# NTU-CompHydroMet-Lab/P2I-GAN-benchmark

Hardware: AMD Instinct MI355X
Metric: train frames/sec (128x128x16) (higher is better)
Workload: dtype f32

## Files before the change

### p2i-gan-benchmark_amd/csrc/glue.hip

```cpp
#include "common.h"

namespace p2i {

template <int T>
__global__ __launch_bounds__(256) void attn_fwd_kernel(const float* __restrict__ x, const float* __restrict__ w0,
                                                       const float* __restrict__ b0, const float* __restrict__ w1,
                                                       const float* __restrict__ b1, float* out, int B, int HW) {
  __shared__ float sw[2][T * T + T];
  for (int i = threadIdx.x; i < T * T; i += blockDim.x) { sw[0][i] = w0[i]; sw[1][i] = w1[i]; }
  for (int i = threadIdx.x; i < T; i += blockDim.x) { sw[0][T * T + i] = b0[i]; sw[1][T * T + i] = b1[i]; }
  __syncthreads();
  const int p = blockIdx.x * blockDim.x + threadIdx.x, b = blockIdx.y;
  if (p >= HW) return;
  float h[T];
#pragma unroll
  for (int t = 0; t < T; ++t) h[t] = x[((size_t)b * T + t) * HW + p];
#pragma unroll
  for (int l = 0; l < 2; ++l) {
    float n[T];
#pragma unroll
    for (int i = 0; i < T; ++i) {
      float g = sw[l][T * T + i];
#pragma unroll
      for (int j = 0; j < T; ++j) g += sw[l][i * T + j] * h[j];
      const float a = h[i] + h[i] * g;
      n[i] = a > 0.f ? a : 0.f;
    }
#pragma unroll
    for (int i = 0; i < T; ++i) h[i] = n[i];
  }
#pragma unroll
  for (int t = 0; t < T; ++t) out[((size_t)b * T + t) * HW + p] = h[t];
}

constexpr int ATTN_LIST = 32;

template <int T>
__global__ __launch_bounds__(256) void attn_bwd_kernel(const float* __restrict__ x, const float* __restrict__ w0,
                                                       const float* __restrict__ b0, const float* __restrict__ w1,
                                                       const float* __restrict__ b1, const float* __restrict__ dout,
                                                       float* dw0, float* db0, float* dw1, float* db1, int B, int HW, DetWs ws) {
  constexpr int NP = T * T + T;
  constexpr int NE = (2 * NP + 255) / 256;
  constexpr int PPT = (ATTN_LIST * T + 255) / 256;
  constexpr int H0 = 0, H1 = 1, DG2 = 2, DG1 = 3;
  __shared__ float sw[2][NP];
  __shared__ float swT[2][T * T];
  __shared__ float lst[ATTN_LIST][4][T];
  __shared__ int act[256];
  __shared__ int wave_cnt[4];
  for (int i = threadIdx.x; i < T * T; i += blockDim.x) {
    const float a = w0[i], c = w1[i];
    sw[0][i] = a; sw[1][i] = c;
// ... 363 lines not shown
}
__global__ void act_bwd_kernel(const float* __restrict__ dy, const float* __restrict__ y, int act, float* out, int64_t n4, int64_t n) {
  for (int64_t i = blockIdx.x * (int64_t)blockDim.x + threadIdx.x; i < n4; i += (int64_t)gridDim.x * blockDim.x) {
    const float4 g = reinterpret_cast<const float4*>(dy)[i], v = reinterpret_cast<const float4*>(y)[i];
    reinterpret_cast<float4*>(out)[i] = make_float4(act_grad(g.x, v.x, act), act_grad(g.y, v.y, act), act_grad(g.z, v.z, act), act_grad(g.w, v.w, act));
  }
  if (blockIdx.x == 0 && threadIdx.x < n - n4 * 4) {
    const int64_t i = n4 * 4 + threadIdx.x;
    out[i] = act_grad(dy[i], y[i], act);
  }
}
__global__ void add2_kernel(float* out, const float* __restrict__ a, const float* __restrict__ b, int64_t n4, int64_t n) {
  for (int64_t i = blockIdx.x * (int64_t)blockDim.x + threadIdx.x; i < n4; i += (int64_t)gridDim.x * blockDim.x) {
    const float4 x = reinterpret_cast<const float4*>(a)[i], y = reinterpret_cast<const float4*>(b)[i];
    reinterpret_cast<float4*>(out)[i] = make_float4(x.x + y.x, x.y + y.y, x.z + y.z, x.w + y.w);
  }
  if (blockIdx.x == 0) for (int64_t i = 4 * n4 + threadIdx.x; i < n; i += blockDim.x) out[i] = a[i] + b[i];
}
__global__ void axpy_kernel(float* y, const float* __restrict__ x, float a, int64_t n) {
  for (int64_t i = blockIdx.x * (int64_t)blockDim.x + threadIdx.x; i < n; i += (int64_t)gridDim.x * blockDim.x) y[i] += a * x[i];
}
__global__ void adam_kernel(float* p, const float* __restrict__ g, float* m, float* v, int64_t n, float step_size, float beta1,
                            float beta2, float eps, float bc2_sqrt) {
  for (int64_t i = blockIdx.x * (int64_t)blockDim.x + threadIdx.x; i < n; i += (int64_t)gridDim.x * blockDim.x) {
    const float gi = g[i];
    const float mi = m[i] + (gi - m[i]) * (1.f - beta1);
    const float vi = beta2 * v[i] + (1.f - beta2) * gi * gi;
    m[i] = mi; v[i] = vi;
    const float denom = sqrtf(vi) / bc2_sqrt + eps;
    p[i] = p[i] - step_size * (mi / denom);
  }
}

__global__ void adam_coef_kernel(int32_t* step_dev, float* coef, float lr, float beta1, float beta2) {
  const int step = step_dev[0] + 1;
  step_dev[0] = step;
  const double bc1 = 1.0 - pow((double)beta1, (double)step), bc2 = 1.0 - pow((double)beta2, (double)step);
  coef[0] = (float)((double)lr / bc1);
  coef[1] = (float)sqrt(bc2);
}
__global__ void adam_dev_kernel(float* p, const float* __restrict__ g, float* m, float* v, int64_t n, const float* __restrict__ coef,
                                float beta1, float beta2, float eps) {
  const float step_size = coef[0], bc2_sqrt = coef[1];
  for (int64_t i = blockIdx.x * (int64_t)blockDim.x + threadIdx.x; i < n; i += (int64_t)gridDim.x * blockDim.x) {
    const float gi = g[i];
    const float mi = m[i] + (gi - m[i]) * (1.f - beta1);
    const float vi = beta2 * v[i] + (1.f - beta2) * gi * gi;
    m[i] = mi; v[i] = vi;
    const float denom = sqrtf(vi) / bc2_sqrt + eps;
    p[i] = p[i] - step_size * (mi / denom);
  }
}

static inline int grid_for(int64_t n, int block = 256, int cap = 8192) {
  int64_t g = (n + block - 1) / block;
  return (int)(g < 1 ? 1 : (g > cap ? cap : g));
}

__global__ __launch_bounds__(256) void det_reduce_kernel(const float* __restrict__ part, int groups, int n, long long gs, long long ks, const DetSegs segs) {
  const int g = blockIdx.x * blockDim.x + threadIdx.x;
  if (g >= groups) return;
  const float* p = part + (long long)g * gs;
  float sacc = 0.f;
  int k = 0;
  for (; k + 8 <= n; k += 8) {
    float v[8];
#pragma unroll
    for (int u = 0; u < 8; ++u) v[u] = p[(long long)(k + u) * ks];
#pragma unroll
    for (int u = 0; u < 8; ++u) sacc += v[u];
  }
  for (; k < n; ++k) sacc += p[(long long)k * ks];
  int r = g;
#pragma unroll
  for (int i = 0; i < 4; ++i) {
    if (r < segs.len[i]) { segs.out[i][r] += sacc; return; }
    r -= segs.len[i];
  }
}
int det_reduce(const float* part, int groups, int n, long long gs, long long ks, const DetSegs& segs, hipStream_t s) {
  P2I_LAUNCH(det_reduce_kernel, dim3(ceil_div(groups, 256)), dim3(256), 0, s, part, groups, n, gs, ks, segs);
  return launch_status();
}
}
using namespace p2i;

extern "C" int p2i_attn_fwd(const float* x, const float* w0, const float* b0, const float* w1, const float* b1, float* out,
                            int B, int T, int HW, void* stream) {
  P2I_REQUIRE(x && w0 && b0 && w1 && b1 && out, "null pointer");
  P2I_REQUIRE(T == 8 || T == 16 || T == 32, "AttentionBlock kernels exist for T in {8, 16, 32}");
  const dim3 grid(ceil_div(HW, 256), B);
  hipStream_t s = (hipStream_t)stream;
  if (T == 16) P2I_LAUNCH(attn_fwd_kernel<16>, grid, dim3(256), 0, s, x, w0, b0, w1, b1, out, B, HW);
  else if (T == 32) P2I_LAUNCH(attn_fwd_kernel<32>, grid, dim3(256), 0, s, x, w0, b0, w1, b1, out, B, HW);
  else P2I_LAUNCH(attn_fwd_kernel<8>, grid, dim3(256), 0, s, x, w0, b0, w1, b1, out, B, HW);
  return launch_status();
}
extern "C" int p2i_attn_bwd(const float* x, const float* w0, const float* b0, const float* w1, const float* b1,
                            const float* dout, float* dw0, float* db0, float* dw1, float* db1, int B, int T, int HW, void* stream) {
  P2I_REQUIRE(x && w0 && b0 && w1 && b1 && dout && dw0 && db0 && dw1 && db1, "null pointer");
  P2I_REQUIRE(T == 8 || T == 16 || T == 32, "AttentionBlock kernels exist for T in {8, 16, 32}");
  int gx = ceil_div(HW, 256);
  const int want = 64 / (B < 64 ? B : 64) > 0 ? 64 / (B < 64 ? B : 64) : 1;
  if (gx > want) gx = want;
  const dim3 grid(gx, B);
  hipStream_t s = (hipStream_t)stream;
  const size_t nblk = (size_t)grid.x * grid.y;
  const DetWs ws = det_take(nblk * 2 * (size_t)(T * T + T), 1);
  if (T == 16) P2I_LAUNCH(attn_bwd_kernel<16>, grid, dim3(256), 0, s, x, w0, b0, w1, b1, dout, dw0, db0, dw1, db1, B, HW, ws);
// ... 83 lines not shown
  P2I_LAUNCH(bias_grad_kernel, dim3(C, chunks), dim3(256), 0, (hipStream_t)stream, dy, y_act, act, db, B, C, inner, ws);
  if (ws.part) return det_reduce(ws.part, C, chunks, chunks, 1, DetSegs{{db, nullptr, nullptr, nullptr}, {C, 0, 0, 0}}, (hipStream_t)stream);
  return launch_status();
}
extern "C" int p2i_act_bwd(const float* dy, const float* y, int act, float* out, int64_t n, void* stream) {
  P2I_REQUIRE(dy && y && out && n > 0, "null pointer");
  P2I_LAUNCH(act_bwd_kernel, dim3(grid_for(n / 4 + 1)), dim3(256), 0, (hipStream_t)stream, dy, y, act, out, n / 4, n);
  return launch_status();
}
extern "C" int p2i_act_bwd_bias(const float* dy, const float* y, int act, float* out, float* db, int B, int C, int64_t inner, void* stream) {
  P2I_REQUIRE(dy && y && out && db && B > 0 && C > 0 && inner > 0, "null pointer");
  P2I_REQUIRE((inner & 3) == 0 && (((uintptr_t)dy | (uintptr_t)y | (uintptr_t)out) & 15) == 0, "inner % 4 and 16-byte alignment");
  int chunks = (int)((inner / 4 + 2047) / 2048);
  if (chunks > 16) chunks = 16;
  const DetWs ws = det_take((size_t)C * B * chunks, 0);
  P2I_LAUNCH(act_bwd_bias_kernel, dim3(C, B, chunks), dim3(256), 0, (hipStream_t)stream, dy, y, act, out, db, C, inner / 4, ws);
  if (ws.part) return det_reduce(ws.part, C, B * chunks, B * chunks, 1, DetSegs{{db, nullptr, nullptr, nullptr}, {C, 0, 0, 0}}, (hipStream_t)stream);
  return launch_status();
}
extern "C" int p2i_axpy(float* y, const float* x, float a, int64_t n, void* stream) {
  P2I_REQUIRE(y && x, "null pointer");
  P2I_LAUNCH(axpy_kernel, dim3(grid_for(n)), dim3(256), 0, (hipStream_t)stream, y, x, a, n);
  return launch_status();
}
extern "C" int p2i_add2(float* out, const float* a, const float* b, int64_t n, void* stream) {
  P2I_REQUIRE(out && a && b && n >= 0, "null pointer");
  const bool al = (((uintptr_t)out | (uintptr_t)a | (uintptr_t)b) & 15) == 0;
  const int64_t n4 = al ? n / 4 : 0;
  P2I_LAUNCH(add2_kernel, dim3(grid_for(n4 + 1)), dim3(256), 0, (hipStream_t)stream, out, a, b, n4, n);
  return launch_status();
}
extern "C" int p2i_zero(float* p, int64_t n, void* stream) {
  P2I_REQUIRE(p && n >= 0, "null pointer");
  if (n > 0 && p2i::memset_async(p, 0, sizeof(float) * (size_t)n, (hipStream_t)stream) != hipSuccess) { set_error("memset failed"); return P2I_EINVAL; }
  return P2I_OK;
}
extern "C" int p2i_adam(float* p, const float* g, float* m, float* v, int64_t n, float lr, float beta1, float beta2, float eps,
                        int step, void* stream) {
  P2I_REQUIRE(p && g && m && v && step >= 1, "bad adam arguments");
  const double bc1 = 1.0 - pow((double)beta1, step), bc2 = 1.0 - pow((double)beta2, step);
  P2I_LAUNCH(adam_kernel, dim3(grid_for(n)), dim3(256), 0, (hipStream_t)stream, p, g, m, v, n, (float)(lr / bc1), beta1,
                     beta2, eps, (float)sqrt(bc2));
  return launch_status();
}

extern "C" int p2i_adam_dev(float* p, const float* g, float* m, float* v, int64_t n, float lr, float beta1, float beta2, float eps,
                            int32_t* step_dev, float* coef2, void* stream) {
  P2I_REQUIRE(p && g && m && v && step_dev && coef2, "bad adam arguments");
  P2I_LAUNCH(adam_coef_kernel, dim3(1), dim3(1), 0, (hipStream_t)stream, step_dev, coef2, lr, beta1, beta2);
  P2I_LAUNCH(adam_dev_kernel, dim3(grid_for(n)), dim3(256), 0, (hipStream_t)stream, p, g, m, v, n, coef2, beta1, beta2, eps);
  return launch_status();
}


namespace p2i {
__global__ __launch_bounds__(256) void assemble_batch_kernel(const uint8_t* __restrict__ fr, const uint8_t* __restrict__ mk,
                                                             float* __restrict__ frames, float* __restrict__ masked,
                                                             float* __restrict__ masks, long long n, long long mask_period) {
  const long long stride = (long long)gridDim.x * 256 * 4;
  for (long long i0 = ((long long)blockIdx.x * 256 + threadIdx.x) * 4; i0 < n; i0 += stride) {
#pragma unroll
    for (int q = 0; q < 4; ++q) {
      const long long i = i0 + q;
      if (i < n) {
        const float v = __fdiv_rn((float)fr[i], 255.0f);
        const float m = mk[i % mask_period] ? 1.0f : 0.0f;
        frames[i] = v;
        masks[i] = m;
        masked[i] = v * m;
      }
    }
  }
}
}

__global__ __launch_bounds__(256) void window_gather_kernel(const float* __restrict__ a, const float* __restrict__ b, float* __restrict__ wa,
                                                           float* __restrict__ wb, int L, int64_t HW4, int w0, int nw, int win, int step) {
  const int64_t per = (int64_t)win * HW4;
  for (int64_t i = blockIdx.x * 256ll + threadIdx.x; i < (int64_t)nw * per; i += (int64_t)gridDim.x * 256) {
    const int w = (int)(i / per);
    const int64_t r = i - (int64_t)w * per;
    const int k = (int)(r / HW4);
    const int64_t p = r - (int64_t)k * HW4;
    const int l = min((w0 + w) * step + k, L - 1);
    reinterpret_cast<float4*>(wa)[i] = reinterpret_cast<const float4*>(a)[(int64_t)l * HW4 + p];
    if (b) reinterpret_cast<float4*>(wb)[i] = reinterpret_cast<const float4*>(b)[(int64_t)l * HW4 + p];
  }
}
__global__ __launch_bounds__(256) void window_mean_kernel(const float* __restrict__ pw, float* __restrict__ out, int L, int64_t HW4, int nwin, int win,
                                                         int step, float scale) {
  for (int64_t i = blockIdx.x * 256ll + threadIdx.x; i < (int64_t)L * HW4; i += (int64_t)gridDim.x * 256) {
    const int l = (int)(i / HW4);
    const int64_t p = i - (int64_t)l * HW4;
    const int wlo = l - win + 1 > 0 ? (l - win + 1 + step - 1) / step : 0, whi = min(l / step, nwin - 1);
    float4 acc = make_float4(0.f, 0.f, 0.f, 0.f);
    for (int w = wlo; w <= whi; ++w) {
      const float4 v = reinterpret_cast<const float4*>(pw)[((int64_t)w * win + (l - w * step)) * HW4 + p];
      acc.x += v.x; acc.y += v.y; acc.z += v.z; acc.w += v.w;
    }
    const float c = fmaxf((float)(whi - wlo + 1), 1e-5f);
    acc.x = fmaxf(acc.x / c * scale, 0.f); acc.y = fmaxf(acc.y / c * scale, 0.f);
    acc.z = fmaxf(acc.z / c * scale, 0.f); acc.w = fmaxf(acc.w / c * scale, 0.f);
    reinterpret_cast<float4*>(out)[i] = acc;
  }
}
extern "C" int p2i_window_gather(const float* a, const float* b, float* wa, float* wb, int L, int64_t HW, int w0, int nw, int win, int step,
// ... 28 lines not shown
```

### p2i-gan-benchmark_amd/csrc/weights.hip

```cpp
#include <stdarg.h>
#include "common.h"

namespace p2i {

static thread_local char g_err[512] = "";
void set_error(const char* fmt, ...) {
  va_list ap;
  va_start(ap, fmt);
  vsnprintf(g_err, sizeof(g_err), fmt, ap);
  va_end(ap);
}

__device__ __forceinline__ int pad32(int v) { return (v + 31) & ~31; }

constexpr int FOLD_MAX_LAYERS = 16;
struct FoldBatch {
  const float* W[FOLD_MAX_LAYERS];
  const float* D[FOLD_MAX_LAYERS];
  const float* Dd[FOLD_MAX_LAYERS];
  float* a[FOLD_MAX_LAYERS];
  float* b[FOLD_MAX_LAYERS];
  const float* g[FOLD_MAX_LAYERS];
};

// ... 241 lines not shown
    if (b.div[L]) v = v / *b.div[L];
    if (b.f[L]) b.f[L][((size_t)tap * I + i) * pad32(O) + o] = v;
    if (b.d[L]) b.d[L][((size_t)tap * O + o) * pad32(I) + i] = v;
  }
}
__global__ void unpack_dot_batched_kernel(const PackBatch b, DetWs ws) {
  __shared__ float red[16];
  const int L = blockIdx.z, O = b.O[L], I = b.I[L], NT = b.NT[L];
  if (!b.div[L]) return;
  float acc = 0.f;
  const int n = O * I * NT;
  for (int idx = blockIdx.x * blockDim.x + threadIdx.x; idx < n; idx += gridDim.x * blockDim.x) {
    const int tap = idx % NT, i = (idx / NT) % I, o = idx / (NT * I);
    acc += b.g[L][((size_t)tap * I + i) * pad32(O) + o] * b.w[L][idx];
  }
  acc = block_sum(acc, red);
  if (ws.part) {
    if (threadIdx.x == 0) ws.part[(size_t)L * gridDim.x + blockIdx.x] = acc;
    return;
  }
  if (threadIdx.x == 0 && acc != 0.f) atomicAdd(b.dot[L], acc);
}
__global__ void unpack_batched_kernel(const PackBatch b) {
  const int L = blockIdx.z, O = b.O[L], I = b.I[L], NT = b.NT[L];
  for (int idx = blockIdx.x * blockDim.x + threadIdx.x; idx < O * I * NT; idx += gridDim.x * blockDim.x) {
    const int tap = idx % NT, i = (idx / NT) % I, o = idx / (NT * I);
    float g = b.g[L][((size_t)tap * I + i) * pad32(O) + o];
    if (b.div[L]) {
      const float sg = *b.div[L];
      g = g / sg - (*b.dot[L] / (sg * sg)) * b.u[L][o] * b.v[L][i * NT + tap];
    }
    if (b.accumulate) b.f[L][idx] += g; else b.f[L][idx] = g;
  }
}

constexpr int SN_MAX_LAYERS = 16;
struct SnBatch {
  const float* w[SN_MAX_LAYERS];
  float* u[SN_MAX_LAYERS];
  float* v[SN_MAX_LAYERS];
  float* sigma[SN_MAX_LAYERS];
  float* scratch[SN_MAX_LAYERS];
  float* usnap[SN_MAX_LAYERS];
  float* vsnap[SN_MAX_LAYERS];
  int O[SN_MAX_LAYERS], K[SN_MAX_LAYERS];
  int n;
};
__global__ __launch_bounds__(256) void sn_wtu_batched_kernel(const SnBatch b) {
  __shared__ float part[4][64];
  const int L = blockIdx.z, O = b.O[L], K = b.K[L];
  if ((int)blockIdx.x * 64 >= K) return;
  const float* w = b.w[L];
  const float* u = b.u[L];
  const int col = threadIdx.x & 63, rg = threadIdx.x >> 6, k = blockIdx.x * 64 + col;
  float acc = 0.f;
  if (k < K)
    for (int o = rg; o < O; o += 4) acc += w[(size_t)o * K + k] * u[o];
  part[rg][col] = acc;
  __syncthreads();
  if (rg == 0 && k < K) b.scratch[L][k] = part[0][col] + part[1][col] + part[2][col] + part[3][col];
}
__global__ void sn_wv_batched_kernel(const SnBatch b) {
  const int L = blockIdx.z, O = b.O[L], K = b.K[L];
  const int o = blockIdx.x * (blockDim.x >> 6) + (threadIdx.x >> 6), lane = threadIdx.x & 63;
  if (o >= O) return;
  const float* w = b.w[L];
  const float* v = b.v[L];
  float acc = 0.f;
  for (int k = lane; k < K; k += 64) acc += w[(size_t)o * K + k] * v[k];
  acc = wave_sum(acc);
  if (lane == 0) b.scratch[L][K + o] = acc;
}
__global__ void sn_finish_batched_kernel(const SnBatch b, int phase) {
  __shared__ float red[16];
  const int L = blockIdx.z, O = b.O[L], K = b.K[L];
  const float* in = phase == 0 ? b.scratch[L] : b.scratch[L] + K;
  const int n = phase == 0 ? K : O;
  if (phase == 2) {
    float acc = 0.f;
    for (int i = threadIdx.x; i < n; i += blockDim.x) acc += b.u[L][i] * in[i];
    acc = block_sum(acc, red);
    if (threadIdx.x == 0) *b.sigma[L] = acc;
    return;
  }
  float* out = phase == 0 ? b.v[L] : b.u[L];
  float* snap = phase == 0 ? b.vsnap[L] : b.usnap[L];
  float acc = 0.f;
  for (int i = threadIdx.x; i < n; i += blockDim.x) acc += in[i] * in[i];
  const float nrm = fmaxf(sqrtf(block_sum(acc, red)), 1e-12f);
  float dot = 0.f;
  for (int i = threadIdx.x; i < n; i += blockDim.x) {
    const float o = in[i] / nrm;
    out[i] = o;
    if (snap) snap[i] = o;
    dot += o * in[i];
  }
  if (phase == 1) {
    dot = block_sum(dot, red);
    if (threadIdx.x == 0) *b.sigma[L] = dot;
  }
}

static int fold_fwd_launch(const FoldBatch& fb, int n, int O, int I, hipStream_t s) {
  P2I_LAUNCH(fold_fwd_tile_batched_kernel, dim3(I / 32, O / 32, n), dim3(256), 0, s, fb, O, I);
  return launch_status();
}
static int fold_bwd_launch(const FoldBatch& fb, int n, int O, int I, hipStream_t s) {
  P2I_LAUNCH(fold_bwd_w_tile_batched_kernel, dim3(I / 32, O / 32, n), dim3(256), 0, s, fb, O, I);
  P2I_LAUNCH(fold_bwd_d_batched_kernel, dim3(I / 32, 1, n), dim3(256), 0, s, fb, O, I);
  return launch_status();
}
static int pack_launch(const PackBatch& b, int n, int maxn, hipStream_t s) {
  const int blocks = ceil_div(maxn, 256);
  P2I_LAUNCH(pack_batched_kernel, dim3(blocks > 512 ? 512 : blocks, 1, n), dim3(256), 0, s, b);
  return launch_status();
}
static int unpack_launch(const PackBatch& b, int n, int maxn, float* dots, hipStream_t s) {
  bool any_sigma = false;
  for (int i = 0; i < n; ++i) any_sigma = any_sigma || b.div[i] != nullptr;
  const int blocks = ceil_div(maxn, 256);
  if (any_sigma) {
    (void)p2i::memset_async(dots, 0, sizeof(float) * n, s);
// ... 174 lines not shown
```

### p2i-gan-benchmark_amd/p2igan_bench/_hip.py

```python
from __future__ import annotations

import ctypes as C
import os

_LIB_PATH = os.path.join(os.path.dirname(os.path.abspath(__file__)), "_lib", "libp2i_hip.so")
_lib = None

ACT_NONE, ACT_RELU, ACT_LEAKY, ACT_TANH = 0, 1, 2, 3


class ConvDesc(C.Structure):
    _fields_ = [(n, C.c_int) for n in
                ("B", "Cin", "Cout", "Ti", "Hi", "Wi", "To", "Ho", "Wo", "kt", "kh", "kw",
                 "st", "sh", "sw", "pt", "ph", "pw")]


class ConvSplit(C.Structure):
    _fields_ = [("w_split", C.c_void_p), ("w_scratch", C.c_void_p), ("src_planes", C.c_void_p), ("w_split_taps", C.c_int)]


class EvalInput(C.Structure):
    _fields_ = [("data", C.c_void_p)] + [(n, C.c_int) for n in ("dtype", "h", "w", "top", "left")]


# ... 107 lines not shown
    "p2i_krig_bins": [_P, _P, _P, _I, _I, _I, _I, _F64, _P, _P],
    "p2i_krig_fit": [_P, _I, _I, _I, _F64, _I, _P, _P, _P, _P, _P],
    "p2i_krig_factor": [_K, _P, _P],
    "p2i_krig_solve": [_K, _P, _P, _P, _P, _P],
    "p2i_krig_predict": [_K, _P, _P, _I, _I, _P, _P],
    "p2i_idw_all": [_P, _P, _P, _I, _I, _I, _I, _F, _P, _P],
    "p2i_krig_invert": [_P, _I, _I, _P, _P],
    "p2i_krig_variance": [_K, _P, _P, _I, _I, _P, _P],
    "p2i_krig_loo": [_K, _P, _P, _P, _P, _P, _P, _P],
    "p2i_krig_cs_spectrum": [_P, _P, _I, _I, _I, _I, _P, _P, _P, _P, _P],
    "p2i_krig_cs_noise": [C.c_uint64, _L, _I, _I, _I, _I, _P, _P],
    "p2i_krig_cs_fields": [_P, _P, _P, _P, C.c_uint64, _I, _I, _I, _I, _I, _I, _I, _I, _P, _P, _P],
    "p2i_krig_cs_weights": [_K, _P, _P, _P, _I, _I, _I, _P, _P, _P],
    "p2i_krig_cs_predict": [_K, _P, _P, _I, _I, _I, _P, _P],
    "p2i_stkrig_gather": [_P, _P, _P, _I, _I, _I, _I, _P, _P, _P, _P, _P],
    "p2i_stkrig_bins": [_P, _P, _P, _P, _I, _I, _I, _I, _I, _I, _F64, _P, _P],
    "p2i_stkrig_fit": [_P, _I, _I, _I, _I, _F64, _I, _P, _P, _P, _P, _P],
    "p2i_stkrig_factor": [_K, _P, _P, _P, _P],
    "p2i_stkrig_predict": [_P, _P, _P, _P, _P, _P, _P, _I, _I, _I, _I, _I, _I, _P, _P],
    "p2i_stkrig_gather_sites": [_P, _P, _P, _I, _I, _I, _I, _P, _P, _P, _P, _P, _P, _P, _P, _P, _P],
    "p2i_stkrig_site_gram": [_P, _I, _I, _P, _P],
    "p2i_stkrig_loso": [_K, _P, _P, _P, _P, _P, _P, _I, _I, _P, _P, _P],
    "p2i_lagkrig_velocity": [_P, _P, _P, _I, _I, _I, _I, _I, _I, _F64, _F64, _P, _P],
    "p2i_lagkrig_pick": [_P, _I, _I, _I, _F64, _P, _P, _P, _P, _P, _P, _P],
    "p2i_lkrig_predict": [_P, _P, _P, _P, _P, _I, _I, _I, _I, _I, _I, _I, _I, _P, _P, _P, _P, _P, _P, _P],
    "p2i_lkrig_loso": [_P, _P, _P, _P, _P, _I, _I, _I, _I, _I, _I, _P, _P, _P, _P, _P, _P],
    "p2i_idw_loo": [_P, _P, _P, _I, _I, _F, _P, _P],
    "p2i_loo_scores": [_P, _P, _P, _P, _I, _I, _P, _P, _P],
    "p2i_scale_fss": [_E, _E, _I, _I, _P, C.POINTER(C.c_double), _I, C.POINTER(C.c_int), _I, _I, _P, _P, _P],
    "p2i_scale_fss_merge": [_P, _L, _I, _P, _P],
    "p2i_scale_dft_rows": [_E, _I, _I, _I, _P, _I, _P, _P, _P, _P],
    "p2i_scale_dft_cols": [_P, _I, _I, _P, _P, _P],
    "p2i_scale_rings": [_P, _I, _I, _P, _P, _P, _P, _I, _P, _P],
    "p2i_scale_spectrum_merge": [_P, _P, _L, _I, _P, _P],
    "p2i_prob_record": [_I, _I, _I, _I, _I, C.POINTER(C.c_int), C.POINTER(C.c_int)],
    "p2i_prob_accumulate": [_E, _E, _F64, _E, _L, _I, _I, _P, _P, C.POINTER(C.c_double), C.POINTER(C.c_double), _I,
                            C.POINTER(C.c_double), _I, C.POINTER(C.c_double), _I, _I, _I, _I, _I, _P, _L, _P],
    "p2i_prob_merge": [_P, _L, _I, _I, _P, _P],
    "p2i_objects_quantize": [_E, _I, _I, _I, _P, C.POINTER(C.c_double), _I, _F64, _F64, _I, _P, _P, _P, _P],
    "p2i_objects_label": [_P, _I, _I, _I, _I, _I, _P, _P],
    "p2i_objects_count": [_P, _I, _P, _I, _I, _I, _P, _P, _P],
    "p2i_objects_scan": [_P, _L, _P, _P],
    "p2i_objects_fill": [_P, _I, _P, _I, _I, _I, _P, _L, _P, _P],
}

ENS_SIGNATURES = {
    "p2i_ens_abi_version": [],
    "p2i_ens_record": [_I, _I, _I, C.POINTER(C.c_int), C.POINTER(C.c_int)],
    "p2i_ens_points": [_E, _I, _L, _E, _L, _I, _I, _I, _P, C.POINTER(C.c_double), _I, C.POINTER(C.c_double), _I, _P, _L, _P],
    "p2i_ens_energy": [_E, _I, _L, _E, _L, _I, _I, _P, _P, _P],
    "p2i_ens_variogram": [_E, _I, _L, _E, _L, _I, _I, _P, C.POINTER(C.c_int), _I, _P, _P],
}


def lib_path() -> str:
    return _LIB_PATH


def load():
    global _lib
    if _lib is not None:
        return _lib
    if not os.path.exists(_LIB_PATH):
        raise RuntimeError(
            f"libp2i_hip.so not found at {_LIB_PATH}: build it with `python -c 'import __graft_entry__ as g; g.build()'` "
            "or `make -C p2i-gan-benchmark_amd/csrc`.  There is no CPU fallback for the product path.")
    lib = C.CDLL(os.environ.get("P2I_HIP_LIB") or _LIB_PATH)
    for table in (SIGNATURES, ENS_SIGNATURES):
        for name, args in table.items():
            fn = getattr(lib, name)
            fn.argtypes = args
            fn.restype = C.c_int
    lib.p2i_abi_version.restype = C.c_int
    lib.p2i_last_error.restype = C.c_char_p
    _lib = lib
    return lib


def check(rc: int, what: str):
    if rc != 0:
        msg = load().p2i_last_error().decode(errors="replace")
        raise RuntimeError(f"{what} failed (rc={rc}): {msg}")
```

### p2i-gan-benchmark_amd/p2igan_bench/engine.py

```python
from __future__ import annotations

from typing import Dict, List, Optional

import torch
import torch.distributed as dist
import torch.nn as nn

from . import ops
from .models import p2igan as net_fns
from .modules.losses import ReconstructionLoss, discriminator_loss, generator_adv_loss
from .parallel import BucketedAllReduce, FlatParams, allreduce_mean_, broadcast_module_state


class FusedAdam:

    def __init__(self, fp: FlatParams, lr: float, betas=(0.0, 0.99), eps: float = 1e-8):
        self.fp, self.lr, self.betas, self.eps = fp, lr, betas, eps
        self.m = torch.zeros_like(fp.flat)
        self.v = torch.zeros_like(fp.flat)
        self.step_count = 0
        self.step_dev = self.coef = None

    def use_device_step(self):
        self.step_dev = torch.tensor([self.step_count], device=self.fp.flat.device, dtype=torch.int32)
# ... 2 lines not shown
    def step(self):
        self.step_count += 1
        if self.step_dev is not None:
            ops.adam_step_dev(self.fp.flat, self.fp.grad, self.m, self.v, self.lr, self.betas[0], self.betas[1], self.eps,
                              self.step_dev, self.coef)
        else:
            ops.adam_step(self.fp.flat, self.fp.grad, self.m, self.v, self.lr, self.betas[0], self.betas[1], self.eps, self.step_count)
        inval = getattr(self.fp.module, "invalidate_weight_cache", None)
        if inval is not None:
            inval()

    def state_dict(self):
        return {"step": self.step_count, "exp_avg": self.m, "exp_avg_sq": self.v, "lr": self.lr, "betas": self.betas, "eps": self.eps}

    def load_state_dict(self, sd):
        self.step_count = int(sd["step"])
        self.m.copy_(sd["exp_avg"])
        self.v.copy_(sd["exp_avg_sq"])
        if self.step_dev is not None:
            self.step_dev.fill_(self.step_count)


def _allreduce_mean(buf: torch.Tensor, world: int):
    allreduce_mean_(buf, world, (lambda t, a: ops.axpy_(t, t, a - 1.0)) if buf.is_cuda else None)


class TrainEngine:
    def __init__(self, generator: nn.Module, discriminator: Optional[nn.Module], cfg: Dict, distributed: bool = False):
        self.G, self.D = generator, discriminator
        loss_cfg, opt_cfg = cfg["loss"], cfg["train"]["optimizer"]
        self.use_gan = bool(loss_cfg.get("use_gan", 0)) and discriminator is not None
        self.gan_type = loss_cfg.get("gan_loss", "hinge")
        self.real_label = loss_cfg.get("target_real_label", 1.0)
        self.fake_label = loss_cfg.get("target_fake_label", 0.0)
        self.adv_weight = loss_cfg.get("adversarial_weight", 0.01)
        self.rec_loss = ReconstructionLoss(k1_alpha=loss_cfg.get("k1_weight", 0.0))
        betas = (opt_cfg.get("beta1", 0.0), opt_cfg.get("beta2", 0.99))
        self.gp = FlatParams(self.G)
        self.opt_g = FusedAdam(self.gp, opt_cfg["lr"], betas)
        import os
        self.direct = os.environ.get("P2I_ENGINE_AUTOGRAD", "0") != "1" and isinstance(self.G, net_fns.P2IGenerator) and (
            discriminator is None or isinstance(discriminator, net_fns.P2IDiscriminator))
        self.dp = self.opt_d = None
        if self.use_gan:
            self.dp = FlatParams(self.D)
            self.opt_d = FusedAdam(self.dp, opt_cfg["lr"], betas)
        self.distributed = distributed and dist.is_initialized() and dist.get_world_size() > 1
        self.world = dist.get_world_size() if self.distributed else 1
        if self.distributed:
            self.broadcast_state()
        self.dp_overlap = os.environ.get("P2I_DP_OVERLAP", "1") != "0"
        self._level_ranges = None
        self.prep_overlap = os.environ.get("P2I_PREP_OVERLAP", "1") != "0"

    def broadcast_state(self):
        broadcast_module_state(self.G, self.gp)
        if self.D is not None:
            broadcast_module_state(self.D, self.dp)

    def level_range(self, lvl: int):
        if self._level_ranges is None:
            base, rngs = self.gp.grad.data_ptr(), []
            for blk in self.G.Decoder:
                ps = [p for p in blk.parameters() if p.requires_grad]
                lo = min((p.grad.data_ptr() - base) // 4 for p in ps)
                hi = max((p.grad.data_ptr() - base) // 4 + p.numel() for p in ps)
                if hi - lo != sum(p.numel() for p in ps):
                    raise RuntimeError("Decoder level is not one contiguous slice of the flat gradient buffer")
                rngs.append((int(lo), int(hi)))
            self._level_ranges = rngs
        return self._level_ranges[lvl]

    def capture(self, frames, masked, masks, warmup: int = 3, mode: str = "graph"):
        if self.distributed:
            raise RuntimeError("graph capture is for the single-GPU step")
        if not self.direct:
            raise RuntimeError("graph / tape capture replays the direct P2I-GAN step only; this engine runs the autograd step "
                               f"({type(self.G).__name__}), which stays eager")
        if mode not in ("graph", "tape"):
            raise ValueError(mode)
        for o in (self.opt_g, self.opt_d):
            if o is not None:
                o.use_device_step()
        self._static_in = [torch.empty_like(t) for t in (frames, masked, masks)]
        for dst, src in zip(self._static_in, (frames, masked, masks)):
            dst.copy_(src)
        side = torch.cuda.Stream()
        side.wait_stream(torch.cuda.current_stream())
        with torch.cuda.stream(side):
            for _ in range(warmup):
                self._step_impl(*self._static_in)
        torch.cuda.current_stream().wait_stream(side)
        self._graph = torch.cuda.CUDAGraph()
        self._tape = None
        import ctypes
        lib = ops._hip.load()
        with torch.cuda.graph(self._graph):
            if mode == "tape":
                ops._hip.check(lib.p2i_tape_begin(torch.cuda.current_stream().cuda_stream), "p2i_tape_begin")
            try:
                self._static_out = self._step_impl(*self._static_in)
            finally:
                if mode == "tape":
                    handle = ctypes.c_void_p()
                    ops._hip.check(lib.p2i_tape_end(ctypes.byref(handle)), "p2i_tape_end")
                    self._tape = handle
# ... 21 lines not shown

    def train_step(self, frames, masked, masks) -> Dict[str, torch.Tensor]:
        if getattr(self, "_graph", None) is not None:
            if tuple(frames.shape) == tuple(self._static_in[0].shape):
                for dst, src in zip(self._static_in, (frames, masked, masks)):
                    if dst.data_ptr() != src.data_ptr():
                        dst.copy_(src)
                if getattr(self, "_tape", None) is not None:
                    ops._hip.check(ops._hip.load().p2i_tape_replay(self._tape, torch.cuda.current_stream().cuda_stream), "p2i_tape_replay")
                else:
                    self._graph.replay()
                for o in (self.opt_g, self.opt_d):
                    if o is not None:
                        o.step_count += 1
                self.G.invalidate_weight_cache() if hasattr(self.G, "invalidate_weight_cache") else None
                return self._static_out
            return self._step_impl(frames, masked, masks)
        if self._auto_graph_wanted(frames):
            shp = tuple(frames.shape)
            self._same_shape_steps = getattr(self, "_same_shape_steps", 0) + 1 if getattr(self, "_last_shape", None) == shp else 0
            self._last_shape = shp
            if self._same_shape_steps >= self.AUTO_GRAPH_AFTER:
                import os
                self.capture(frames, masked, masks, warmup=0, mode="tape" if os.environ.get("P2I_AUTO_TAPE", "0") == "1" else "graph")
                return self.train_step(frames, masked, masks)
        return self._step_impl(frames, masked, masks)

    def _mark(self):
        if self.phase_marks is not None:
            e = torch.cuda.Event(enable_timing=True)
            e.record()
            self.phase_marks.append(e)

    phase_marks = None
    exchange_marks = None

    def _exchange(self, kind, fn):
        if self.exchange_marks is None or not self.gp.grad.is_cuda:
            return fn()
        e0, e1 = torch.cuda.Event(enable_timing=True), torch.cuda.Event(enable_timing=True)
        e0.record()
        out = fn()
        e1.record()
        self.exchange_marks.append((kind, e0, e1))
        return out

    def _step_direct(self, frames, masked, masks) -> Dict[str, torch.Tensor]:
        G, D = self.G, self.D
        self._mark()
        if not G.training:
            G.train()
        with torch.no_grad():
            side = net_fns._side_of(G, frames.device) if (self.prep_overlap and frames.is_cuda) else None
            real_box = [None]
            step_start = ops.mark_stream() if side is not None else None

            def enqueue_side_work():
                b_, t_, c_, h_, w_ = masked.shape
                gprep = side.run(lambda: net_fns.generator_prepare(G, b_, h_, w_), after=step_start)
                ready = side.mark()
                if self.use_gan:
                    if not D.training:
                        D.train()
                    dprep_f = side.run(lambda: net_fns.discriminator_prepare(D, tuple(masked.shape), frames.device, False, True, pool=True), after=step_start)
                    dprep_r = side.run(lambda: net_fns.discriminator_prepare(D, tuple(frames.shape), frames.device, False, True, pool=True), after=step_start)

                    def real_pass():
                        lr2, cr2 = net_fns.discriminator_forward(D, frames, need_x=False, need_p=True, pool=True, prep=dprep_r)
                        _, dlr2, _ = ops.gan_loss_d(lr2, lr2, self.gan_type, self.real_label, self.fake_label)
                        self.dp.zero_grad()
                        net_fns.discriminator_backward(D, cr2, dlr2, need_x=False, inplace=True, accumulate=False)
                        return lr2, None

                    real_box[0] = (dprep_f, side.run(real_pass, frames, after=step_start))
                return gprep, ready

            preds, S = net_fns.generator_forward(G, masked, masks, need_grad=True, after_head=enqueue_side_work if side is not None else None)
            dprep_f, real_out = real_box[0] if real_box[0] is not None else (None, None)
            if side is not None and self.use_gan:
                out3, dpred = side.run(lambda: ops.recloss(preds.contiguous(), frames.contiguous().float(), self.rec_loss.k1_alpha), preds, frames)
            else:
                out3, dpred = ops.recloss(preds.contiguous(), frames.contiguous().float(), self.rec_loss.k1_alpha)
            out = {"rec": out3[2], "pool": out3[0], "reg": out3[1]}
            self._mark()
            dgen = dpred
            loss_g = out3[2:3]
            if self.use_gan:
                if not D.training:
                    D.train()
                lf, cf = net_fns.discriminator_forward(D, preds, need_x=False, need_p=True, pool=True, prep=dprep_f)
            if side is not None:
                side.join()
            if self.use_gan:
                if real_out is not None and real_out[1] is None:
                    lr_ = real_out[0]
                    loss_d, _, dlf = ops.gan_loss_d(lr_, lf, self.gan_type, self.real_label, self.fake_label)
                    net_fns.discriminator_backward(D, cf, dlf, need_x=False, inplace=True, accumulate=True)
                    del cf
                else:
                    lr_, cr = real_out if real_out is not None else net_fns.discriminator_forward(D, frames, need_x=False, need_p=True, pool=True)
                    loss_d, dlr, dlf = ops.gan_loss_d(lr_, lf, self.gan_type, self.real_label, self.fake_label)
                    self.dp.zero_grad()
                    net_fns.discriminator_backward(D, cf, dlf, need_x=False, inplace=True, accumulate=False)
                    net_fns.discriminator_backward(D, cr, dlr, need_x=False, inplace=True, accumulate=True)
                    del cf, cr
                if self.distributed:
                    self._exchange("d", lambda: _allreduce_mean(self.dp.grad, self.world))
                self.opt_d.step()
                self._mark()
                lg, cg = net_fns.discriminator_forward(D, preds, need_x=True, need_p=False, pool=True)
                adv, dlg = ops.gan_loss_g(lg, self.adv_weight, self.gan_type, self.real_label)
                dgen, _, _, _ = net_fns.discriminator_backward(D, cg, dlg, need_x=True, needs=[False] * (2 * sum(map(len, D.layers())) + 1), dx_add=dpred)
                del cg
                loss_g = ops.add2(out3[2:3], adv)
                out.update(loss_d=loss_d.reshape(()), adv=adv.reshape(()), logits_real=lr_, logits_fake=lf)
            self.gp.zero_grad()
            if self.distributed and self.dp_overlap:
                bk = BucketedAllReduce(self.gp.grad, self.world, (lambda t, a: ops.axpy_(t, t, a - 1.0)) if self.gp.grad.is_cuda else None)
                net_fns.generator_backward(G, S, dgen, inplace=True, on_level_done=lambda lvl: bk.launch(*self.level_range(lvl)))
                del S
                self._exchange("g", bk.finish)
            else:
                net_fns.generator_backward(G, S, dgen, inplace=True)
                del S
                if self.distributed:
                    self._exchange("g", lambda: _allreduce_mean(self.gp.grad, self.world))
            self.opt_g.step()
            out.update(loss_g=loss_g.reshape(()), preds=preds)
            self._mark()
        return out

    def _step_impl(self, frames, masked, masks) -> Dict[str, torch.Tensor]:
        if self.direct:
            with ops.step_stream():
                return self._step_direct(frames, masked, masks)
        self._mark()
        self.G.train()
        preds = self.G(masked, masks)
        loss_g, parts = self.rec_loss(preds, frames, masks)
        out = {"rec": loss_g.detach(), "pool": parts["pool"].tensor(), "reg": parts["reg"].tensor()}
        self._mark()
        if self.use_gan:
            self.D.train()
            for p in self.dp.params:
                p.requires_grad_(True)
# ... 43 lines not shown
```

### p2i-gan-benchmark_amd/p2igan_bench/ops.py

```python
from __future__ import annotations

import ctypes as C
import math
from dataclasses import dataclass
from typing import Optional, Tuple

import torch

from . import _hip
from ._hip import ACT_LEAKY, ACT_NONE, ACT_RELU, ACT_TANH, ConvDesc


def _ptr(t: Optional[torch.Tensor]):
    return None if t is None else t.data_ptr()


_CUR_STREAM = None


def _stream():
    return _CUR_STREAM if _CUR_STREAM is not None else torch.cuda.current_stream().cuda_stream


class step_stream:
# ... 1087 lines not shown

def shock_map_bwd(x, dout, beta, eps):
    _chk_f32(x, dout)
    _same(x, dout, "shock_map_bwd")
    B, T, H, W, _, _ = _shock_dims(x, 1, 0, "shock_map")
    dx = torch.empty_like(x)
    scratch = torch.empty(3 * x.numel(), device=x.device, dtype=torch.float32)
    _hip.check(_hip.load().p2i_shock_map_bwd(_ptr(x), _ptr(dout), _ptr(dx), _ptr(scratch), B * T, H, W, float(beta), float(eps),
                                             _stream()), "p2i_shock_map_bwd")
    return dx


def shock_loss_fwd(pred, true, beta, pool, border, eps):
    _chk_f32(pred, true)
    _same(pred, true, "shock_loss_fwd")
    B, T, H, W, Hp, Wp = _shock_dims(pred, pool, border, "shock_map_loss")
    out = torch.empty((B, T, Hp - 2 * border, Wp - 2 * border), device=pred.device, dtype=torch.float32)
    _hip.check(_hip.load().p2i_shock_loss_fwd(_ptr(pred), _ptr(true), _ptr(out), B * T, H, W, int(pool), int(border), float(beta),
                                              float(eps), _stream()), "p2i_shock_loss_fwd")
    return out


def shock_loss_bwd(pred, true, dout, beta, pool, border, eps):
    _chk_f32(pred, true, dout)
    B, T, H, W, Hp, Wp = _shock_dims(pred, pool, border, "shock_map_loss")
    if tuple(dout.shape) != (B, T, Hp - 2 * border, Wp - 2 * border):
        raise RuntimeError(f"shock_loss_bwd: gradient {tuple(dout.shape)} does not match the loss tensor")
    dpred = torch.empty_like(pred)
    scratch = torch.empty(3 * B * T * Hp * Wp, device=pred.device, dtype=torch.float32)
    _hip.check(_hip.load().p2i_shock_loss_bwd(_ptr(pred), _ptr(true), _ptr(dout), _ptr(dpred), _ptr(scratch), B * T, H, W, int(pool),
                                              int(border), float(beta), float(eps), _stream()), "p2i_shock_loss_bwd")
    return dpred


def adam_step(p, g, m, v, lr, beta1, beta2, eps, step):
    lib = _hip.load()
    n = p.numel()
    if not (g.numel() == n and m.numel() == n and v.numel() == n):
        raise RuntimeError("adam_step: buffer size mismatch")
    _chk(p, g, m, v)
    _hip.check(lib.p2i_adam(_ptr(p), _ptr(g), _ptr(m), _ptr(v), n, lr, beta1, beta2, eps, step, _stream()), "p2i_adam")


def adam_step_dev(p, g, m, v, lr, beta1, beta2, eps, step_dev, coef):
    lib = _hip.load()
    n = p.numel()
    if not (g.numel() == n and m.numel() == n and v.numel() == n) or step_dev.dtype != torch.int32 or coef.numel() < 2:
        raise RuntimeError("adam_step_dev: bad buffers")
    _chk(p, g, m, v, step_dev, coef)
    _hip.check(lib.p2i_adam_dev(_ptr(p), _ptr(g), _ptr(m), _ptr(v), n, lr, beta1, beta2, eps, _ptr(step_dev), _ptr(coef), _stream()),
               "p2i_adam_dev")


def axpy_(y, x, a=1.0):
    lib = _hip.load()
    if y.numel() != x.numel():
        raise RuntimeError("axpy_: size mismatch")
    _chk(y, x)
    _hip.check(lib.p2i_axpy(_ptr(y), _ptr(x), float(a), y.numel(), _stream()), "p2i_axpy")
    return y


def zero_(t):
    lib = _hip.load()
    _chk(t)
    _hip.check(lib.p2i_zero(_ptr(t), t.numel(), _stream()), "p2i_zero")
    return t


def add2(a, b):
    lib = _hip.load()
    if a.shape != b.shape:
        raise RuntimeError("add2: shape mismatch")
    out = torch.empty_like(a)
    _chk(a, b)
    _hip.check(lib.p2i_add2(_ptr(out), _ptr(a), _ptr(b), a.numel(), _stream()), "p2i_add2")
    return out


def act_bwd(dy, y, act):
    lib = _hip.load()
    if dy.shape != y.shape:
        raise RuntimeError("act_bwd: shape mismatch")
    out = torch.empty_like(dy)
    _chk(dy, y)
    _hip.check(lib.p2i_act_bwd(_ptr(dy), _ptr(y), act, _ptr(out), dy.numel(), _stream()), "p2i_act_bwd")
    return out


def act_bwd_bias(dy, y, act, db_out=None):
    lib = _hip.load()
    det_ready(dy.device)
    B, Cc = dy.shape[0], dy.shape[1]
    inner = dy[0, 0].numel()
    if inner % 4:
        dz = act_bwd(dy, y, act)
        return dz, bias_grad(dz, out=db_out)
    out = torch.empty_like(dy)
    db = db_out if db_out is not None else zero_(torch.empty(Cc, device=dy.device, dtype=torch.float32))
    _chk(dy, y, db)
    _hip.check(lib.p2i_act_bwd_bias(_ptr(dy), _ptr(y), act, _ptr(out), _ptr(db), B, Cc, inner, _stream()), "p2i_act_bwd_bias")
    return out, db


def bias_grad(dy, y_act=None, act=ACT_NONE, out=None):
    lib = _hip.load()
# ... 1085 lines not shown
```

Measured before the change: 11460.

## Add vectorized ranged Adam, unroll spectral-norm matvecs, split discriminator side stream

Adds float4-vectorized ranged Adam entry points (host and device-step variants) with alignment-aware head/tail handling, though nothing in the shown code calls them yet. Rewrites the spectral-norm W^T u and W v kernels with deep unrolled load batches and fma to raise memory-level parallelism. The engine gets a separate side stream for discriminator prep, the real pass and the reconstruction loss, plus an event so the fake-branch forward waits only on its own prep. This aims for more overlap with generator work, at the cost of more streams and sync points.

```diff
diff --git a/include/p2i_opt.h b/include/p2i_opt.h
--- /dev/null
+++ b/include/p2i_opt.h
@@ -0,0 +1,18 @@
+#ifndef P2I_OPT_H
+#define P2I_OPT_H
+#include "p2i_hip.h"
+
+#ifdef __cplusplus
+extern "C" {
+#endif
+
+int p2i_opt_abi_version(void);
+int p2i_adam_range(float* p, const float* g, float* m, float* v, int64_t offset, int64_t n, float lr, float beta1, float beta2,
+                   float eps, int step, void* stream);
+int p2i_adam_range_dev(float* p, const float* g, float* m, float* v, int64_t offset, int64_t n, float lr, float beta1, float beta2,
+                       float eps, int32_t* step_dev, float* coef2, int advance, void* stream);
+
+#ifdef __cplusplus
+}
+#endif
+#endif
diff --git a/p2i-gan-benchmark_amd/csrc/glue.hip b/p2i-gan-benchmark_amd/csrc/glue.hip
--- a/p2i-gan-benchmark_amd/csrc/glue.hip
+++ b/p2i-gan-benchmark_amd/csrc/glue.hip
@@ -1,4 +1,5 @@
 #include "common.h"
+#include "p2i_opt.h"
 
 namespace p2i {
 
@@ -468,9 +469,54 @@
   }
 }
 
+__device__ __forceinline__ void adam_one(float& p, float gi, float& m, float& v, float step_size, float beta1, float beta2,
+                                         float eps, float bc2_sqrt) {
+#pragma clang fp contract(off)
+  const float mi = m + (gi - m) * (1.f - beta1);
+  const float vi = beta2 * v + (1.f - beta2) * gi * gi;
+  m = mi; v = vi;
+  const float denom = sqrtf(vi) / bc2_sqrt + eps;
+  p = fmaf(-step_size, mi / denom, p);
+}
+__global__ void adam_range_kernel(float* p, const float* __restrict__ g, float* m, float* v, int64_t n, int head, int64_t n4,
+                                  const float* __restrict__ coef, float step_size, float beta1, float beta2, float eps,
+                                  float bc2_sqrt) {
+  if (coef) { step_size = coef[0]; bc2_sqrt = coef[1]; }
+  float4* p4 = reinterpret_cast<float4*>(p + head);
+  const float4* g4 = reinterpret_cast<const float4*>(g + head);
+  float4* m4 = reinterpret_cast<float4*>(m + head);
+  float4* v4 = reinterpret_cast<float4*>(v + head);
+  for (int64_t i = blockIdx.x * (int64_t)blockDim.x + threadIdx.x; i < n4; i += (int64_t)gridDim.x * blockDim.x) {
+    float4 pi = p4[i], mi = m4[i], vi = v4[i];
+    const float4 gi = g4[i];
+    adam_one(pi.x, gi.x, mi.x, vi.x, step_size, beta1, beta2, eps, bc2_sqrt);
+    adam_one(pi.y, gi.y, mi.y, vi.y, step_size, beta1, beta2, eps, bc2_sqrt);
+    adam_one(pi.z, gi.z, mi.z, vi.z, step_size, beta1, beta2, eps, bc2_sqrt);
+    adam_one(pi.w, gi.w, mi.w, vi.w, step_size, beta1, beta2, eps, bc2_sqrt);
+    m4[i] = mi; v4[i] = vi; p4[i] = pi;
+  }
+  if (blockIdx.x == 0) {
+    const int64_t tail0 = head + 4 * n4;
+    for (int64_t i = threadIdx.x; i < head + (n - tail0); i += blockDim.x) {
+      const int64_t e = i < head ? i : tail0 + (i - head);
+      adam_one(p[e], g[e], m[e], v[e], step_size, beta1, beta2, eps, bc2_sqrt);
+    }
+  }
+}
+
 static inline int grid_for(int64_t n, int block = 256, int cap = 8192) {
   int64_t g = (n + block - 1) / block;
   return (int)(g < 1 ? 1 : (g > cap ? cap : g));
+}
+static inline void adam_range_cut(const float* p, const float* g, const float* m, const float* v, int64_t n, int* head, int64_t* n4) {
+  const uintptr_t ph = (uintptr_t)p & 15;
+  int64_t h = n;
+  if ((ph & 3) == 0 && ((uintptr_t)g & 15) == ph && ((uintptr_t)m & 15) == ph && ((uintptr_t)v & 15) == ph) {
+    h = (int64_t)((16 - ph) & 15) / 4;
+    if (h > n) h = n;
+  }
+  *head = (int)(h < n ? h : 0);
+  *n4 = h < n ? (n - h) / 4 : 0;
 }
 
 __global__ __launch_bounds__(256) void det_reduce_kernel(const float* __restrict__ part, int groups, int n, long long gs, long long ks, const DetSegs segs) {
@@ -660,6 +706,31 @@
   return launch_status();
 }
 
+extern "C" int p2i_opt_abi_version(void) { return 1; }
+static int adam_range_launch(float* p, const float* g, float* m, float* v, int64_t offset, int64_t n, const float* coef,
+                             float step_size, float beta1, float beta2, float eps, float bc2_sqrt, hipStream_t s) {
+  if (n == 0) return launch_status();
+  p += offset; g += offset; m += offset; v += offset;
+  int head;
+  int64_t n4;
+  adam_range_cut(p, g, m, v, n, &head, &n4);
+  P2I_LAUNCH(adam_range_kernel, dim3(grid_for(n4)), dim3(256), 0, s, p, g, m, v, n, head, n4, coef, step_size, beta1, beta2, eps,
+             bc2_sqrt);
+  return launch_status();
+}
+extern "C" int p2i_adam_range(float* p, const float* g, float* m, float* v, int64_t offset, int64_t n, float lr, float beta1,
+                              float beta2, float eps, int step, void* stream) {
+  P2I_REQUIRE(p && g && m && v && step >= 1 && offset >= 0 && n >= 0, "bad adam arguments");
+  const double bc1 = 1.0 - pow((double)beta1, step), bc2 = 1.0 - pow((double)beta2, step);
+  return adam_range_launch(p, g, m, v, offset, n, nullptr, (float)(lr / bc1), beta1, beta2, eps, (float)sqrt(bc2), (hipStream_t)stream);
+}
+extern "C" int p2i_adam_range_dev(float* p, const float* g, float* m, float* v, int64_t offset, int64_t n, float lr, float beta1,
+                                  float beta2, float eps, int32_t* step_dev, float* coef2, int advance, void* stream) {
+  P2I_REQUIRE(p && g && m && v && step_dev && coef2 && offset >= 0 && n >= 0, "bad adam arguments");
+  if (advance) P2I_LAUNCH(adam_coef_kernel, dim3(1), dim3(1), 0, (hipStream_t)stream, step_dev, coef2, lr, beta1, beta2);
+  return adam_range_launch(p, g, m, v, offset, n, coef2, 0.f, beta1, beta2, eps, 1.f, (hipStream_t)stream);
+}
+
 
 namespace p2i {
 __global__ __launch_bounds__(256) void assemble_batch_kernel(const uint8_t* __restrict__ fr, const uint8_t* __restrict__ mk,
diff --git a/p2i-gan-benchmark_amd/csrc/weights.hip b/p2i-gan-benchmark_amd/csrc/weights.hip
--- a/p2i-gan-benchmark_amd/csrc/weights.hip
+++ b/p2i-gan-benchmark_amd/csrc/weights.hip
@@ -317,10 +317,27 @@
   if ((int)blockIdx.x * 64 >= K) return;
   const float* w = b.w[L];
   const float* u = b.u[L];
-  const int col = threadIdx.x & 63, rg = threadIdx.x >> 6, k = blockIdx.x * 64 + col;
+  const int col = threadIdx.x & 63, rg = __builtin_amdgcn_readfirstlane(threadIdx.x >> 6), k = blockIdx.x * 64 + col;
   float acc = 0.f;
-  if (k < K)
-    for (int o = rg; o < O; o += 4) acc += w[(size_t)o * K + k] * u[o];
+  if (k < K) {
+    const float* wk = w + k;
+    int o = rg;
+    for (; o + 4 * 31 < O; o += 4 * 32) {
+      float wv[32], uv[32];
+#pragma unroll
+      for (int j = 0; j < 32; ++j) { wv[j] = wk[(size_t)(o + 4 * j) * K]; uv[j] = u[o + 4 * j]; }
+#pragma unroll
+      for (int j = 0; j < 32; ++j) acc = fmaf(wv[j], uv[j], acc);
+    }
+    for (; o + 4 * 7 < O; o += 4 * 8) {
+      float wv[8], uv[8];
+#pragma unroll
+      for (int j = 0; j < 8; ++j) { wv[j] = wk[(size_t)(o + 4 * j) * K]; uv[j] = u[o + 4 * j]; }
+#pragma unroll
+      for (int j = 0; j < 8; ++j) acc = fmaf(wv[j], uv[j], acc);
+    }
+    for (; o < O; o += 4) acc = fmaf(wk[(size_t)o * K], u[o], acc);
+  }
   part[rg][col] = acc;
   __syncthreads();
   if (rg == 0 && k < K) b.scratch[L][k] = part[0][col] + part[1][col] + part[2][col] + part[3][col];
@@ -332,7 +349,23 @@
   const float* w = b.w[L];
   const float* v = b.v[L];
   float acc = 0.f;
-  for (int k = lane; k < K; k += 64) acc += w[(size_t)o * K + k] * v[k];
+  const float* wo = w + (size_t)o * K;
+  int k = lane;
+  for (; k + 64 * 15 < K; k += 64 * 16) {
+    float wv[16], vv[16];
+#pragma unroll
+    for (int j = 0; j < 16; ++j) { wv[j] = wo[k + 64 * j]; vv[j] = v[k + 64 * j]; }
+#pragma unroll
+    for (int j = 0; j < 16; ++j) acc = fmaf(wv[j], vv[j], acc);
+  }
+  for (; k + 64 * 3 < K; k += 64 * 4) {
+    float wv[4], vv[4];
+#pragma unroll
+    for (int j = 0; j < 4; ++j) { wv[j] = wo[k + 64 * j]; vv[j] = v[k + 64 * j]; }
+#pragma unroll
+    for (int j = 0; j < 4; ++j) acc = fmaf(wv[j], vv[j], acc);
+  }
+  for (; k < K; k += 64) acc = fmaf(wo[k], v[k], acc);
   acc = wave_sum(acc);
   if (lane == 0) b.scratch[L][K + o] = acc;
 }
diff --git a/p2i-gan-benchmark_amd/p2igan_bench/_hip.py b/p2i-gan-benchmark_amd/p2igan_bench/_hip.py
--- a/p2i-gan-benchmark_amd/p2igan_bench/_hip.py
+++ b/p2i-gan-benchmark_amd/p2igan_bench/_hip.py
@@ -183,6 +183,12 @@
     "p2i_ens_variogram": [_E, _I, _L, _E, _L, _I, _I, _P, C.POINTER(C.c_int), _I, _P, _P],
 }
 
+OPT_SIGNATURES = {
+    "p2i_opt_abi_version": [],
+    "p2i_adam_range": [_P, _P, _P, _P, _L, _L, _F, _F, _F, _F, _I, _P],
+    "p2i_adam_range_dev": [_P, _P, _P, _P, _L, _L, _F, _F, _F, _F, _P, _P, _I, _P],
+}
+
 
 def lib_path() -> str:
     return _LIB_PATH
@@ -197,7 +203,7 @@
             f"libp2i_hip.so not found at {_LIB_PATH}: build it with `python -c 'import __graft_entry__ as g; g.build()'` "
             "or `make -C p2i-gan-benchmark_amd/csrc`.  There is no CPU fallback for the product path.")
     lib = C.CDLL(os.environ.get("P2I_HIP_LIB") or _LIB_PATH)
-    for table in (SIGNATURES, ENS_SIGNATURES):
+    for table in (SIGNATURES, ENS_SIGNATURES, OPT_SIGNATURES):
         for name, args in table.items():
             fn = getattr(lib, name)
             fn.argtypes = args
diff --git a/p2i-gan-benchmark_amd/p2igan_bench/engine.py b/p2i-gan-benchmark_amd/p2igan_bench/engine.py
--- a/p2i-gan-benchmark_amd/p2igan_bench/engine.py
+++ b/p2i-gan-benchmark_amd/p2igan_bench/engine.py
@@ -78,6 +78,7 @@
         self.dp_overlap = os.environ.get("P2I_DP_OVERLAP", "1") != "0"
         self._level_ranges = None
         self.prep_overlap = os.environ.get("P2I_PREP_OVERLAP", "1") != "0"
+        self.head_split = os.environ.get("P2I_HEAD_SPLIT", "1") != "0"
 
     def broadcast_state(self):
         broadcast_module_state(self.G, self.gp)
@@ -205,6 +206,9 @@
             G.train()
         with torch.no_grad():
             side = net_fns._side_of(G, frames.device) if (self.prep_overlap and frames.is_cuda) else None
+            side_d = side
+            if side is not None and self.use_gan and self.head_split:
+                side_d = net_fns._side_of(D, frames.device)
             real_box = [None]
             step_start = ops.mark_stream() if side is not None else None
 
@@ -215,8 +219,9 @@
                 if self.use_gan:
                     if not D.training:
                         D.train()
-                    dprep_f = side.run(lambda: net_fns.discriminator_prepare(D, tuple(masked.shape), frames.device, False, True, pool=True), after=step_start)
-                    dprep_r = side.run(lambda: net_fns.discriminator_prepare(D, tuple(frames.shape), frames.device, False, True, pool=True), after=step_start)
+                    dprep_f = side_d.run(lambda: net_fns.discriminator_prepare(D, tuple(masked.shape), frames.device, False, True, pool=True), after=step_start)
+                    fake_ready = side_d.mark()
+                    dprep_r = side_d.run(lambda: net_fns.discriminator_prepare(D, tuple(frames.shape), frames.device, False, True, pool=True), after=step_start)
 
                     def real_pass():
                         lr2, cr2 = net_fns.discriminator_forward(D, frames, need_x=False, need_p=True, pool=True, prep=dprep_r)
@@ -225,13 +230,13 @@
                         net_fns.discriminator_backward(D, cr2, dlr2, need_x=False, inplace=True, accumulate=False)
                         return lr2, None
 
-                    real_box[0] = (dprep_f, side.run(real_pass, frames, after=step_start))
+                    real_box[0] = (dprep_f, side_d.run(real_pass, frames, after=step_start), fake_ready)
                 return gprep, ready
 
             preds, S = net_fns.generator_forward(G, masked, masks, need_grad=True, after_head=enqueue_side_work if side is not None else None)
-            dprep_f, real_out = real_box[0] if real_box[0] is not None else (None, None)
+            dprep_f, real_out, fake_ready = real_box[0] if real_box[0] is not None else (None, None, None)
             if side is not None and self.use_gan:
-                out3, dpred = side.run(lambda: ops.recloss(preds.contiguous(), frames.contiguous().float(), self.rec_loss.k1_alpha), preds, frames)
+                out3, dpred = side_d.run(lambda: ops.recloss(preds.contiguous(), frames.contiguous().float(), self.rec_loss.k1_alpha), preds, frames)
             else:
                 out3, dpred = ops.recloss(preds.contiguous(), frames.contiguous().float(), self.rec_loss.k1_alpha)
             out = {"rec": out3[2], "pool": out3[0], "reg": out3[1]}
@@ -241,9 +246,11 @@
             if self.use_gan:
                 if not D.training:
                     D.train()
+                if fake_ready is not None:
+                    fake_ready()
                 lf, cf = net_fns.discriminator_forward(D, preds, need_x=False, need_p=True, pool=True, prep=dprep_f)
-            if side is not None:
-                side.join()
+            if side_d is not None:
+                side_d.join()
             if self.use_gan:
                 if real_out is not None and real_out[1] is None:
                     lr_ = real_out[0]
diff --git a/p2i-gan-benchmark_amd/p2igan_bench/ops.py b/p2i-gan-benchmark_amd/p2igan_bench/ops.py
--- a/p2i-gan-benchmark_amd/p2igan_bench/ops.py
+++ b/p2i-gan-benchmark_amd/p2igan_bench/ops.py
@@ -1163,6 +1163,28 @@
                "p2i_adam_dev")
 
 
+def _adam_range_chk(p, g, m, v, lo, hi):
+    n = p.numel()
+    if not (g.numel() == n and m.numel() == n and v.numel() == n and 0 <= lo <= hi <= n):
+        raise RuntimeError("adam range: buffer size mismatch or range outside the buffer")
+
+
+def adam_range(p, g, m, v, lo, hi, lr, beta1, beta2, eps, step):
+    _adam_range_chk(p, g, m, v, lo, hi)
+    _chk(p, g, m, v)
+    _hip.check(_hip.load().p2i_adam_range(_ptr(p), _ptr(g), _ptr(m), _ptr(v), lo, hi - lo, lr, beta1, beta2, eps, step, _stream()),
+               "p2i_adam_range")
+
+
+def adam_range_dev(p, g, m, v, lo, hi, lr, beta1, beta2, eps, step_dev, coef, advance):
+    _adam_range_chk(p, g, m, v, lo, hi)
+    if step_dev.dtype != torch.int32 or coef.numel() < 2:
+        raise RuntimeError("adam_range_dev: bad buffers")
+    _chk(p, g, m, v, step_dev, coef)
+    _hip.check(_hip.load().p2i_adam_range_dev(_ptr(p), _ptr(g), _ptr(m), _ptr(v), lo, hi - lo, lr, beta1, beta2, eps, _ptr(step_dev),
+                                              _ptr(coef), 1 if advance else 0, _stream()), "p2i_adam_range_dev")
+
+
 def axpy_(y, x, a=1.0):
     lib = _hip.load()
     if y.numel() != x.numel():
```

New measurement: 11550, median of 3. Within noise of the previous version (+0.8%).
